# maiziezhoulab/FocalSV

Measured on AMD Instinct MI355X. Metric: target regions/sec (50 kb, 30x HiFi), higher is better.
Workload: dtype u32; 1 GPU; 256 synthetic 50 kb regions per GPU, 30x HiFi-like reads U(10k,20k), 0.2% error, seed 1000+i (BASELINE.json configs[1]); regions_per_gpu=256

## Files before the change

### focalsv_amd/csrc/aln.hip

```cpp
#include "k_sketch.h"
#include <algorithm>
#include <memory>
#include <cstdio>
#include <cstdlib>
#include <cstring>
#include <vector>

namespace {

#define ALN_AMAX 8192
#define ALN_CHAIN_STRIDE (ALN_AMAX + 8)
#define ALN_MAX_REC 5
#define ALN_MAJ_REC 3
#define ALN_SUP_MIN 200
#define ALN_SUB_OCC 2
#define ALN_SUB_PER 1500
#define ALN_EV_CAP 2048
#define ALN_CG_CAP 1024
#define NW_LDS_Q 3072
#define NW_NEG (-(1 << 29))

struct AlnHeader { int32_t qbeg, tbeg, qend, tend, n_events, n_chain, rev, status; uint32_t ev_off, pad; };
struct AlnEvent { int32_t qs, qe, ts, te; };
struct NwTask { uint32_t pair; int32_t qs, ql, ts, tl; uint32_t cg_off; uint64_t bt_off; uint64_t row_off; uint32_t out_idx, pad; };
// ... 675 lines not shown
__global__ __launch_bounds__(256) void k_nw_any(const uint32_t *__restrict__ store, const uint32_t *__restrict__ nm_all, const uint32_t *__restrict__ word_off,
                                                const int32_t *__restrict__ read_len, const uint32_t *__restrict__ pair_q,
                                                const uint32_t *__restrict__ pair_t, const AlnHeader *__restrict__ hdr,
                                                const NwTask *__restrict__ tasks, uint8_t *__restrict__ bt_all, int32_t *__restrict__ rows_all,
                                                uint32_t *__restrict__ cg_all, uint32_t *__restrict__ cg_n, int32_t *__restrict__ scores, fsv_aln_params P)
{
    const uint32_t *nm = nm_active(nm_all);
    __shared__ uint8_t s_bt[NW_TD][NW_TC];
    __shared__ int s_walk[8];
    const NwTask T = tasks[blockIdx.x];
    const uint32_t qw = word_off[pair_q[T.pair]], tw = word_off[pair_t[T.pair]];
    const int lenq = read_len[pair_q[T.pair]], rev = hdr[T.pair].rev;
    const int ql = T.ql, tl = T.tl;
    const bool two = P.q2 >= 0;
    const NwRows R{rows_all + T.row_off, ql};
    uint8_t *bt = bt_all + T.bt_off;
    for (int d = 0; d <= ql + tl - 2; d++) {
        const int jlo = max(0, d - (tl - 1)), jhi = min(ql - 1, d);
        for (int j = jlo + (int)threadIdx.x; j <= jhi; j += blockDim.x) {
            const int i = d - j;
            nw_cell(R, d, i, j, tbase(store, nm, tw, T.ts + i), qbase(store, qw, lenq, rev, T.qs + j), two, P, bt, ql);
        }
        __threadfence_block();
        __syncthreads();
    }
    if (threadIdx.x == 0) scores[T.out_idx] = R.H(ql + tl - 2)[ql - 1];
    nw_backtrack(bt, ql, tl, cg_all + T.cg_off, cg_n + T.out_idx, s_bt, s_walk);
}

struct NwLanes {
    hipStream_t side[3] = {nullptr, nullptr, nullptr};
    hipEvent_t fork = nullptr, join[3] = {nullptr, nullptr, nullptr};
    NwLanes() = default;
    NwLanes(const NwLanes &) = delete;
    NwLanes &operator=(const NwLanes &) = delete;
    ~NwLanes()
    {
        for (int i = 0; i < 3; i++) { if (side[i]) (void)hipStreamDestroy(side[i]); if (join[i]) (void)hipEventDestroy(join[i]); }
        if (fork) (void)hipEventDestroy(fork);
    }
    int ready(fsv_ctx *ctx)
    {
        if (fork) return FSV_OK;
        FSV_HIP(ctx, hipEventCreateWithFlags(&fork, hipEventDisableTiming));
        for (int i = 0; i < 3; i++) {
            FSV_HIP(ctx, hipStreamCreateWithFlags(&side[i], hipStreamNonBlocking));
            FSV_HIP(ctx, hipEventCreateWithFlags(&join[i], hipEventDisableTiming));
        }
        return FSV_OK;
    }
};

struct AlnWs {
    Dev<uint32_t> store, word_off, pair_q, pair_t, sk_ends, sk_low, sk_high, mz_off, mz_cnt, warn, ev_count, cg, cg_n;
    Dev<uint32_t> nmask;
    Dev<int32_t> len, rows, scores, gap_shift;
    Dev<char> ascii;
    Dev<uint64_t> asc_off, chain;
    Dev<uint8_t> wper, bt;
    Dev<uint16_t> thin;
    Dev<fsv_mz> mz;
    Dev<AlnHeader> hdr;
    Dev<AlnEvent> events, ev_packed;
    Dev<NwTask> tasks;
    Dev<GapQuery> gaps;
    Dev<BoxSrc> box_src;
    Dev<CornerTask> corner;
    Dev<int2> corner_out;
    fsv_aln_stats stats = {};
    NwLanes lanes;
    std::unique_ptr<AlnWs> sub;
    const uint32_t *nm() const { return nmask.p + FSV_NM_LEAD; }
};

void aln_ws_free(fsv_ctx *ctx)
{
    delete (AlnWs *)ctx->aln_ws;
    ctx->aln_ws = nullptr;
}

AlnWs *aln_ws_get(fsv_ctx *ctx)
{
    if (!ctx->aln_ws) { ctx->aln_ws = new AlnWs(); ctx->aln_ws_free = aln_ws_free; }
    return (AlnWs *)ctx->aln_ws;
}

#define PAIR_SEQS(W) (W).store.p, (W).nm(), (W).word_off.p, (W).len.p, (W).pair_q.p, (W).pair_t.p
template <class K, class... A> int launch_pair(fsv_ctx *ctx, const AlnWs &W, hipStream_t stream, K kern, size_t grid, uint32_t block, A... own)
{
    FSV_LAUNCH(ctx, stream, kern, dim3((uint32_t)grid), dim3(block), 0, PAIR_SEQS(W), W.hdr.p, own...);
    return FSV_OK;
}
template <bool SUB> int launch_chain_aln(fsv_ctx *ctx, const AlnWs &W, uint32_t np, uint32_t R, const fsv_aln_params &P)
{
    FSV_LAUNCH(ctx, ctx->stream, k_chain_aln<SUB>, dim3(np), dim3(64), 0, W.len.p, W.mz.p, W.mz_off.p, W.mz_cnt.p, W.pair_q.p, W.pair_t.p, W.chain.p, W.hdr.p, R, P);
    return FSV_OK;
}
template <bool SUB> int launch_events(fsv_ctx *ctx, const AlnWs &W, uint32_t ns, const fsv_aln_params &P)
{
    FSV_LAUNCH(ctx, ctx->stream, k_aln_events<SUB>, dim3(ns), dim3(256), 0, PAIR_SEQS(W), W.chain.p, W.hdr.p, W.events.p, W.ev_packed.p, W.ev_count.p, P);
    return FSV_OK;
}

template <class L, class F> int lay_out(fsv_ctx *ctx, const std::vector<L> &len, F unit, uint64_t slack, std::vector<uint32_t> &off)
{
    const size_t n = len.size();
    off.assign(n + 1, 0);
// ... 602 lines not shown
```

### focalsv_amd/csrc/asm.hip

```cpp
#include "asm_kernels.h"
#include "k_kmer.h"
#include "layout.h"
#include <algorithm>
#include <chrono>
#include <cstdio>
#include <cstdlib>
#include <cstring>
#include <vector>
#include <thread>
#include <atomic>

namespace {

enum { KN_SKETCH, KN_UNIQ, KN_CHAIN, KN_BPM, KN_RESCUE, KN_PATH_FAST, KN_PATH_DP, KN_CONSENSUS, KN_REPACK, KN_EXACT, KN_STITCH, KN_PARTITION, KN_BND, KN_BND_CONS, KN_COUNT,
       ST_SKETCH = KN_COUNT, ST_CHAIN, ST_VERIFY, ST_PATH, ST_CONSENSUS, ST_FINAL };
const char *const kn_names[KN_COUNT] = {"k_sketch", "k_uniq", "k_chain", "k5_bpm", "k_rescue_accept", "k_path_fast", "k_path_dp", "k_consensus",
                                        "k_repack", "k_exact", "k_stitch", "k_partition", "k_bnd_tasks", "k_bnd_consensus"};
enum { PASS_NONE = -1, PASS_WINDOWS, PASS_JUNCTIONS, PASS_BCIG, PASS_COUNT };

struct KTimes {
    struct Rec { int k; hipEvent_t a, b; uint64_t bytes; };
    std::vector<Rec> recs;
    std::vector<hipEvent_t> pool;
    size_t used = 0;
    std::vector<size_t> by[PASS_COUNT][KN_COUNT];
    hipEvent_t get() { if (used == pool.size()) { hipEvent_t e; (void)hipEventCreate(&e); pool.push_back(e); } return pool[used++]; }
    size_t begin(fsv_ctx *ctx, int k, uint64_t bytes) { Rec r{k, get(), get(), bytes}; (void)hipEventRecord(r.a, ctx->stream); recs.push_back(r); return recs.size() - 1; }
    void begin(fsv_ctx *ctx, int pass, int k, uint64_t bytes) { const size_t i = begin(ctx, k, bytes); if (pass != PASS_NONE) by[pass][k].push_back(i); }
    void end(fsv_ctx *ctx) { (void)hipEventRecord(recs.back().b, ctx->stream); }
    void end(fsv_ctx *ctx, size_t idx) { (void)hipEventRecord(recs[idx].b, ctx->stream); }
    uint64_t *bytes_of(int pass, int k, size_t round) { const auto &v = by[pass][k]; return round < v.size() ? &recs[v[round]].bytes : nullptr; }
    void reset() { recs.clear(); used = 0; for (auto &p : by) for (auto &v : p) v.clear(); }
    ~KTimes() { for (auto e : pool) (void)hipEventDestroy(e); }
};

struct Span {
    fsv_ctx *ctx; KTimes &kt; size_t idx;
    Span(fsv_ctx *c, KTimes &k, int stage) : ctx(c), kt(k), idx(k.begin(c, stage, 0)) {}
    void stop() { kt.end(ctx, idx); }
};

enum { CT_TASKS = 0, CT_OVERFLOW = 1, CT_DP = 2, CT_INEXACT = 3, CT_COLS_LO = 4, CT_COLS_HI = 5, CT_DP_WIDE = 6, CT_DP_SB = 7, CT_DP_GEN = 8, CT_DP_XW = 9,
       CT_MZ_LO = 10, CT_MZ_HI = 11, CT_B_RETRY = 12, CT_B_LIST = 13, CT_DP_SB16 = 14, CT_WIDE = 15,
       CT_MZRAW_LO = 16, CT_MZRAW_HI = 17, CT_BASES_LO = 18, CT_BASES_HI = 19,
       CT_DP_FR3 = 20,
       CT_LEFT = 21,
       CT_FIX = 22, CT_FIXED = 23,
       CT_SLOT = 24 };

template <class... Ts> size_t cap_sum(const Ts &...b) { return (b.cap + ... + 0); }

struct AsmWs {
    Dev<uint32_t> store[2], word_off, set_start, read_set, pair_base, upair_base, pair_read, mz_off, mz_cnt, counters, warn, set_cols, changed, read_dirty,
        dp_list, dp_list2, dp_list3, dp_list16, dp_list_e3, dp_wide, dp_xwide, left_list, fix_list, wide_list, inexact_list, cols_wide,
        gwin_off, gwin_read, lb, unpack_off, brel_off, src3, bnd_flag, bnd_list, site_cnt, site_off, redo, sk_ends, sk_low, sk_high;
    Dev<uint32_t> sr_store;
    Dev<uint32_t> site_cursor;
    Dev<uint32_t> site_lists;
    Dev<uint32_t> set_hits;
    Dev<int32_t> len, new_len, idx2, bc_idx;
    Dev<int32_t> bc_win;
    Dev<fsv_mz> mz; Dev<fsv_ovl> ovl, ovl_prev; Dev<fsv_hit> hits, hits_packed; Dev<fsv_piece> pieces; Dev<BndPatch> bnd_patch;
    Dev<fsv_wtask> tasks, tasks2, tasks3; Dev<fsv_wres> res, res2, res3; Dev<fsv_wpath> paths, paths2;
    Dev<uint4> cols_sb, ovl_c, upair_tab, upair_tab_sw, gwin_tab, bc_rec; Dev<uint2> site_rec; Dev<int8_t> site_vec;
    Dev<uint64_t> cols;
    Dev<unsigned long long> tmp;
    Dev<uint8_t> cov3, bnd_bytes, exact_flag, cwin, thr_tab; Dev<uint16_t> cwin_len; Dev<char> contig_out, contig_all;
    Dev<unsigned long long> km_keys, km_flt, km_flt_all; Dev<uint32_t> km_cnt, km_hist, km_cursor, km_err; Dev<uint64_t> km_tab_off, km_flt_off;
    Dev<int32_t> km_cutoff; Dev<KmerTile> km_tiles;
    Dev<unsigned long long> fs_keys, fs_list; Dev<uint64_t> fs_off, fs_list_off; Dev<uint32_t> fs_read_set;
    SketchFilter flt;
    std::vector<fsv_kmer_index_set> ki_last; double ki_ms = 0; bool ki_valid = false;
    Dev<fsv_wtask> ext_tasks; Dev<fsv_wext> ext_res; Dev<uint32_t> ext_list, charge_list, charge_n; Dev<unsigned long long> charge_ct;
    std::vector<hipEvent_t> charge_ev;
    fsv_charge_stats charge_last{};
    bool charge_valid = false;
    std::vector<fsv_kmer_set> km_last; std::vector<uint64_t> km_last_flt_off; const unsigned long long *km_last_flt = nullptr; double km_ms = 0; bool km_valid = false;
    std::vector<uint32_t> h_store;
    int occ_sb = 0, occ_fr[3] = {0, 0, 0}, occ_wide = 0;
    ChainArgs last_chain;
    std::vector<uint32_t> h_word_off;
    std::vector<int32_t> h_len;
    const uint32_t *cur_store = nullptr;
    uint32_t n_reads = 0;
    fsv_asm_stats stats;
    KTimes kt;
    void *h_pin = nullptr; size_t h_pin_cap = 0;
    uint32_t *ct_of(int row) { return counters.p + (size_t)row * CT_SLOT; }
    size_t held() const
    {
        return cap_sum(store[0], store[1], cols_sb, contig_all, word_off, len, set_start, read_set, pair_base, mz, mz_off, mz_cnt, ovl, tasks, res, paths,
                       counters, dp_list, dp_list2, dp_list3, dp_list16, dp_list_e3, dp_wide, dp_xwide, cols_wide, set_cols, site_cnt, site_rec, site_off, site_vec,
                       site_cursor, redo, site_lists, read_dirty, cov3, lb, sr_store, brel_off, tasks2, res2, paths2, idx2, bc_idx, bc_rec, bc_win, left_list, fix_list,
                       tasks3, res3, src3, bnd_flag, bnd_list, bnd_patch, bnd_bytes, changed, pair_read, wide_list, cols, tmp, gwin_off, gwin_read, sk_ends, sk_low, sk_high,
                       hits, hits_packed, set_hits, ovl_prev, exact_flag, inexact_list, upair_base, upair_tab, upair_tab_sw, ovl_c, gwin_tab, cwin, cwin_len, warn, thr_tab,
                       pieces, contig_out, new_len, unpack_off, km_keys, km_flt, km_flt_all, km_cnt, km_hist, km_cursor, km_err, km_tab_off, km_flt_off, km_cutoff, km_tiles,
                       fs_keys, fs_list, fs_off, fs_list_off, fs_read_set, ext_tasks, ext_res, ext_list, charge_list, charge_n, charge_ct);
    }
};

void ws_free(fsv_ctx *ctx)
{
    AsmWs *w = (AsmWs *)ctx->asm_ws;
    if (!w) return;
    if (w->h_pin) (void)hipHostFree(w->h_pin);
    for (auto e : w->charge_ev) (void)hipEventDestroy(e);
    delete w;
    ctx->asm_ws = nullptr;
}

AsmWs *ws_get(fsv_ctx *ctx)
{
    if (!ctx->asm_ws) { ctx->asm_ws = new AsmWs(); ctx->asm_ws_free = ws_free; memset(&((AsmWs *)ctx->asm_ws)->stats, 0, sizeof(fsv_asm_stats)); }
    return (AsmWs *)ctx->asm_ws;
}

uint8_t thr_for_len_host(int x_len, int rate_pm)
{
    const double rate = rate_pm / 1000.0;
    if (x_len == FSV_WINDOW) return rate_pm == 40 ? FSV_K_FULL : (uint8_t)(int)(FSV_WINDOW * rate);
    int t = (int)(x_len * rate);
    if (t == 0 && x_len >= 4) t = 1;
    return (uint8_t)t;
}

struct Batch {
    uint32_t n_reads = 0, n_sets = 0, n_pairs = 0, n_upairs = 0;
    std::vector<uint32_t> set_start, read_set, pair_base, upair_base;
};

struct Geometry {
    std::vector<uint32_t> word_off, mz_off, gwin_off, gwin_read;
    uint64_t task_bound = 0;
    uint32_t max_words = 1;
};

static inline uint64_t mz_slots(int64_t len, int) { return (uint64_t)len + 64; }

int make_geometry(fsv_ctx *ctx, const Batch &B, const std::vector<int32_t> &len, Geometry &G, int mz_w = 51, const std::vector<uint32_t> *fixed_mz_off = nullptr)
{
    G.word_off.assign(B.n_reads + 1, 0); G.mz_off.assign(B.n_reads + 1, 0); G.gwin_off.assign(B.n_reads + 1, 0);
    G.max_words = 1;
    uint64_t w = 0, m = 0, g = 0;
    for (uint32_t r = 0; r < B.n_reads; r++) {
        G.word_off[r] = (uint32_t)w; G.mz_off[r] = (uint32_t)m; G.gwin_off[r] = (uint32_t)g;
        w += (uint64_t)(len[r] + 15) / 16;
        G.max_words = std::max<uint32_t>(G.max_words, (uint32_t)((len[r] + 15) / 16));
// ... 1394 lines not shown
}

static int check_asm_params(fsv_ctx *ctx, const fsv_asm_params &P)
{
    if (P.k < 1 || P.k > 63 || P.w < 1 || P.w > 64 || P.lookback != 64 || P.n_rounds < 0 || P.n_rounds > 16 || P.min_anchors < 1)
        return fsv_fail(ctx, FSV_EINVAL, "fsv_asm_params out of range (k<=63, w<=64, lookback==64)");
    if (P.k_cap < 1 || P.k_cap > FSV_K_WIDE || P.win_rate_pm < 1 || (int)(FSV_WINDOW * (P.win_rate_pm / 1000.0)) > P.k_cap || P.accept_err_pm < 0 || P.accept_err_pm > 1000 ||
        P.w_later < 0 || P.w_later > 64)
        return fsv_fail(ctx, FSV_EINVAL, "fsv_asm_params error model out of range (k_cap <= 95, 375 x win_rate_pm / 1000 <= k_cap)");
    if (P.kmer_filter && !P.kmer_table)
        return fsv_fail(ctx, FSV_EINVAL, "kmer_filter = 1 needs kmer_table = 1: the filter is the list the k-mer count table stage leaves");
    if (P.partial_charge && P.k_cap > FSV_K_MAX)
        return fsv_fail(ctx, FSV_EINVAL, "partial_charge needs k_cap <= 31 (FSV_K_MAX): the charge is not restated for the wide-band profiles");
    return FSV_OK;
}

static int fsv_assemble_batch_impl(fsv_ctx *ctx, const fsv_readsets *sets, const fsv_asm_params *params, fsv_contigs *out)
{
    if (!ctx || !sets || !out || !sets->store_dev || !sets->word_off || !sets->read_len || !sets->set_start) return FSV_EINVAL;
    if (!out->seq || !out->off || !out->set || !out->n_reads || !out->set_status) return FSV_EINVAL;
    fsv_asm_params P;
    if (params) P = *params; else fsv_asm_default_params(&P);
    TRY(check_asm_params(ctx, P));
    FSV_HIP(ctx, hipSetDevice(ctx->device));
    AsmWs &W = *ws_get(ctx);
    out->n_contigs = 0; out->off[0] = 0;
    W.km_last.clear(); W.km_last_flt_off.assign(1, 0); W.km_last_flt = nullptr; W.km_ms = 0; W.km_valid = false;
    W.flt = SketchFilter{}; W.ki_last.clear(); W.ki_ms = 0; W.ki_valid = false;
    W.charge_last = fsv_charge_stats{}; W.charge_valid = false;
    for (auto e : W.charge_ev) (void)hipEventDestroy(e);
    W.charge_ev.clear();
    if (sets->n_sets == 0 || (sets->n_reads == 0 && !P.kmer_table)) { for (uint32_t s = 0; s < sets->n_sets; s++) out->set_status[s] = 0; memset(&W.stats, 0, sizeof(W.stats)); W.charge_valid = P.partial_charge != 0; return FSV_OK; }
    if (sets->set_start[0] != 0 || sets->set_start[sets->n_sets] != sets->n_reads) return fsv_fail(ctx, FSV_EINVAL, "set_start must span [0, n_reads]");
    for (uint32_t s = 0; s < sets->n_sets; s++) if (sets->set_start[s + 1] < sets->set_start[s]) return fsv_fail(ctx, FSV_EINVAL, "set_start not monotone");
    const char *env = getenv("FSV_ASM_BUDGET_GB");
    double budget = 0.4 * (double)ctx->hbm_bytes;
    {
        size_t free_b = 0, total_b = 0;
        const size_t own = W.held();
        if (hipMemGetInfo(&free_b, &total_b) == hipSuccess)
            budget = std::min(budget, 0.9 * ((double)free_b / (double)std::max(1, fsv_live_contexts(ctx->device)) + (double)own));
    }
    if (env && atof(env) > 0) budget = atof(env) * 1e9;
    std::vector<uint32_t> cut{0};
    {
        uint64_t tk = 0, pr = 0, bs = 0, km = 0;
        for (uint32_t s = 0; s < sets->n_sets; s++) {
            uint64_t t1, p1, b1, k1, f1;
            set_cost(sets, s, t1, p1, b1, k1, f1);
            if (!P.kmer_table) k1 = 0;
            if (P.kmer_filter) k1 += f1;
            if (t1 >= (1ull << 31) || p1 >= (1ull << 31) || b1 + b1 / 4 >= (1ull << 32)) return fsv_fail(ctx, FSV_EUNSUP, "a single read set exceeds the 2^31 window-task / pair bound");
            const bool over = tk + t1 >= (1ull << 31) || pr + p1 >= (1ull << 31) || (bs + b1) + (bs + b1) / 4 >= (1ull << 32) ||
                              (double)(tk + t1) * (P.second_round ? 400.0 : 200.0) + (double)(pr + p1) * 200.0 + (double)(bs + b1) * (P.second_round ? 52.0 : 48.0) +
                              (double)(km + k1) + (P.partial_charge ? (double)(tk + t1) * 104.0 : 0.0) > budget;
            if (over && s > cut.back()) { cut.push_back(s); tk = pr = bs = km = 0; }
            tk += t1; pr += p1; bs += b1; km += k1;
        }
        cut.push_back(sets->n_sets);
    }
    if (cut.size() == 2) { TRY(assemble_chunk(ctx, sets, P, out)); W.km_valid = P.kmer_table != 0; W.ki_valid = P.kmer_filter != 0; W.charge_valid = P.partial_charge != 0; return FSV_OK; }
    fsv_asm_stats total; memset(&total, 0, sizeof(total));
    uint64_t used = 0; uint32_t nc = 0;
    std::vector<uint64_t> all_off{0};
    for (size_t c = 0; c + 1 < cut.size(); c++) {
        const uint32_t s0 = cut[c], s1 = cut[c + 1], r0 = sets->set_start[s0], r1 = sets->set_start[s1];
        std::vector<uint32_t> sub_start(s1 - s0 + 1);
        for (uint32_t s = s0; s <= s1; s++) sub_start[s - s0] = sets->set_start[s] - r0;
        fsv_readsets sub = *sets;
        std::vector<uint64_t> sub_woff((size_t)(r1 - r0) + 1);
        for (uint32_t r = r0; r <= r1; r++) sub_woff[r - r0] = sets->word_off[r] - sets->word_off[r0];
        sub.store_dev = sets->store_dev + sets->word_off[r0];
        sub.word_off = sub_woff.data(); sub.read_len = sets->read_len + r0; sub.set_start = sub_start.data();
        sub.n_reads = r1 - r0; sub.n_sets = s1 - s0; sub.set_flags = sets->set_flags ? sets->set_flags + s0 : nullptr;
        fsv_contigs part = *out;
        part.seq = out->seq + used; part.seq_cap = out->seq_cap - used; part.off = out->off + nc; part.set = out->set + nc; part.n_reads = out->n_reads + nc;
        part.contig_cap = out->contig_cap - nc; part.set_status = out->set_status + s0; part.n_contigs = 0;
        const uint64_t keep = out->off[nc];
        TRY(assemble_chunk(ctx, &sub, P, &part));
        out->off[nc] = keep;
        for (uint32_t i = 0; i < part.n_contigs; i++) { out->set[nc + i] += s0; out->off[nc + i + 1] += used; }
        const uint64_t bytes = part.n_contigs ? out->off[nc + part.n_contigs] - used : 0;
        if (bytes) {
            if (W.contig_all.cap < used + bytes + 16) {
                Dev<char> bigger;
                TRY(ensure(ctx, bigger, std::max<uint64_t>((used + bytes) * 2, 1u << 20)));
                if (used) FSV_HIP(ctx, hipMemcpyAsync(bigger.p, W.contig_all.p, used, hipMemcpyDeviceToDevice, ctx->stream));
                FSV_HIP(ctx, hipStreamSynchronize(ctx->stream));
                W.contig_all.swap(bigger);
            }
            FSV_HIP(ctx, hipMemcpyAsync(W.contig_all.p + used, W.contig_out.p, bytes, hipMemcpyDeviceToDevice, ctx->stream));
        }
        used += bytes; nc += part.n_contigs;
        const fsv_asm_stats &st = W.stats;
        total.n_pairs += st.n_pairs; total.n_overlaps += st.n_overlaps; total.n_windows += st.n_windows; total.n_windows_matched += st.n_windows_matched;
        total.n_paths += st.n_paths; total.n_path_dp += st.n_path_dp; total.dp_columns += st.dp_columns; total.algo_bytes += st.algo_bytes;
        total.n_exact_overlaps += st.n_exact_overlaps; total.n_inexact_candidates += st.n_inexact_candidates; total.n_path_fr += st.n_path_fr;
        total.ms_sketch += st.ms_sketch; total.ms_chain += st.ms_chain; total.ms_verify += st.ms_verify; total.ms_path += st.ms_path;
        total.ms_consensus += st.ms_consensus; total.ms_final += st.ms_final; total.ms_total += st.ms_total;
        total.n_kernels = st.n_kernels;
        for (uint32_t k = 0; k < st.n_kernels; k++) {
            memcpy(total.kernels[k].name, st.kernels[k].name, sizeof(st.kernels[k].name));
            total.kernels[k].ms += st.kernels[k].ms; total.kernels[k].launches += st.kernels[k].launches; total.kernels[k].algo_bytes += st.kernels[k].algo_bytes;
        }
    }
    FSV_HIP(ctx, hipStreamSynchronize(ctx->stream));
    out->n_contigs = nc;
// ... 218 lines not shown
```

### focalsv_amd/csrc/k_sketch.h

```cpp
#pragma once
#include "fsv_internal.h"

#define FSV_UQ_MAX     4096

namespace {

__device__ __forceinline__ uint64_t mix64(uint64_t key)
{
    key = ~key + (key << 21);
    key = key ^ key >> 24;
    key = (key + (key << 3)) + (key << 8);
    key = key ^ key >> 14;
    key = (key + (key << 2)) + (key << 4);
    key = key ^ key >> 28;
    key = key + (key << 31);
    return key;
}

#ifndef FSV_KMER_EMPTY
#define FSV_KMER_EMPTY (~0ull)
#endif
template <bool FLT> struct FltView {};
template <> struct FltView<true> { const unsigned long long *keys; const uint64_t *off; const uint32_t *read_set; };
struct SketchFilter { const unsigned long long *keys = nullptr; const uint64_t *off = nullptr; const uint32_t *read_set = nullptr; };
// ... 220 lines not shown
    __syncthreads();
    const uint32_t m = mz_cnt[r];
    const uint32_t o0 = s_scan[tid];
    const uint32_t slot_cap = mz_off[r + 1] - mz_off[r];
    __syncthreads();
#pragma unroll
    for (uint32_t j = 0; j < UQ_MAX / 256; j++)
        if (j < cnt) { s_hash[o0 + j] = kh[j]; s_pay[o0 + j] = kp[j]; }
    __syncthreads();
    for (uint32_t i = tid; i < m; i += 256) { fsv_mz x; x.hash = s_hash[i]; const uint64_t p = s_pay[i]; x.pos = (uint32_t)p; x.rev = (uint8_t)(p >> 32); x.span = (uint8_t)(p >> 40); x.pad = 0; a[i] = x; }
    if (2 * m <= slot_cap) {
        uint32_t mp = 1;
        while (mp < m) mp <<= 1;
        for (uint32_t i = m + tid; i < mp; i += 256) { s_hash[i] = ~0ull; s_pay[i] = ~0ull; }
        __syncthreads();
        for (uint32_t sz = 2; sz <= mp; sz <<= 1)
            for (uint32_t st = sz >> 1; st > 0; st >>= 1) {
                for (uint32_t t = tid; t < mp / 2; t += 256) {
                    const uint32_t i = ((t & ~(st - 1)) << 1) | (t & (st - 1)), j = i | st;
                    const bool up = (i & sz) == 0;
                    const uint64_t pi = s_pay[i], pj = s_pay[j];
                    bool gt = (uint32_t)pi > (uint32_t)pj || ((uint32_t)pi == (uint32_t)pj && pi > pj);
                    if (pi == ~0ull && pj != ~0ull) gt = true; else if (pj == ~0ull) gt = false;
                    if (gt == up) { const uint64_t hi2 = s_hash[i], hj = s_hash[j]; s_hash[i] = hj; s_hash[j] = hi2; s_pay[i] = pj; s_pay[j] = pi; }
                }
                __syncthreads();
            }
        for (uint32_t i = tid; i < m; i += 256) { fsv_mz x; x.hash = s_hash[i]; const uint64_t p = s_pay[i]; x.pos = (uint32_t)p; x.rev = (uint8_t)(p >> 32); x.span = (uint8_t)(p >> 40); x.pad = 0; a[m + i] = x; }
    } else if (tid == 0) atomicOr(&warn[r], (uint32_t)FSV_W_INTERNAL);
}

template <int UQ_MAX>
__global__ __launch_bounds__(256) void k_uniq(fsv_mz *__restrict__ mz, const uint32_t *__restrict__ mz_off, uint32_t *__restrict__ mz_cnt,
                                              uint32_t *__restrict__ warn, const uint32_t *__restrict__ only_changed = nullptr,
                                              uint32_t lo_cnt = 0u, uint32_t hi_cnt = 0xffffffffu, unsigned long long *__restrict__ total = nullptr,
                                              uint32_t max_occ = 1u)
{
    uniq_read<UQ_MAX>(blockIdx.x, mz, mz_off, mz_cnt, warn, only_changed, lo_cnt, hi_cnt, total, max_occ);
}

template <int UQ_MAX>
__global__ __launch_bounds__(256) void k_uniq_walk(fsv_mz *__restrict__ mz, const uint32_t *__restrict__ mz_off, uint32_t *__restrict__ mz_cnt,
                                                   uint32_t *__restrict__ warn, const uint32_t *__restrict__ only_changed, uint32_t lo_cnt, uint32_t hi_cnt,
                                                   unsigned long long *__restrict__ total, uint32_t n_reads)
{
    for (uint32_t r = blockIdx.x; r < n_reads; r += gridDim.x) {
        uniq_read<UQ_MAX>(r, mz, mz_off, mz_cnt, warn, only_changed, lo_cnt, hi_cnt, total);
        __syncthreads();
    }
}

#define SKF_T 1024
#define SKF_V ((SKF_T + 2 * 256 + 255) / 256)
template <bool FLT>
__global__ __launch_bounds__(256) void k_sketch_fast(const uint32_t *__restrict__ store, const uint32_t *__restrict__ word_off,
                                                     const int32_t *__restrict__ read_len, const uint32_t *__restrict__ mz_off,
                                                     fsv_mz *__restrict__ mz, uint32_t *__restrict__ mz_cnt, uint32_t n_reads, int w, int k,
                                                     int hpc, uint32_t *__restrict__ warn, const uint8_t *__restrict__ w_per_read,
                                                     uint32_t *__restrict__ sc_ends, uint32_t *__restrict__ sc_low, uint32_t *__restrict__ sc_high,
                                                     const uint32_t *__restrict__ only_changed, const FltView<FLT> F)
{
    __shared__ uint64_t s_h[SKF_T + 2 * 256];
    __shared__ uint64_t s_wmin[SKF_T + 2 * 256];
    __shared__ uint32_t s_scan[4];
    __shared__ uint32_t s_carry;
    __shared__ uint64_t s_am, s_ah;
    __shared__ int s_abest, s_short;
    const int tid = threadIdx.x;
    const uint32_t r = blockIdx.x;
    if (r >= n_reads) return;
    if (only_changed && !only_changed[r]) return;
    const uint32_t woff = word_off[r];
    const int len = read_len[r];
    const uint32_t cap = mz_off[r + 1] - mz_off[r];
    fsv_mz *out = mz + mz_off[r];
    if (w_per_read) w = w_per_read[r];
    [[maybe_unused]] uint64_t fbase = 0, fsize = 0;
    if constexpr (FLT) { const uint32_t fs = F.read_set[r]; fbase = F.off[fs]; fsize = F.off[fs + 1] - fbase; }
    if (tid == 0) mz_cnt[r] = 0;
    uint32_t *ends = sc_ends + (size_t)woff * 16;
    uint32_t *low = sc_low + woff + r, *high = sc_high + woff + r;
    const uint64_t NONE = ~0ull;
    const uint64_t kmask = (1ull << k) - 1;
    const int nwords = (len + 15) >> 4;
    if (tid == 0) s_carry = 0;
    __syncthreads();
    for (int wbase = 0; wbase < nwords; wbase += 256) {
        const int wi = wbase + tid;
        uint32_t flags = 0, word = 0;
        int nb = 0;
        if (wi < nwords) {
            word = store[woff + wi];
            nb = min(16, len - wi * 16);
            if (hpc) {
                const uint32_t nextb = (wi + 1 < nwords) ? (store[woff + wi + 1] & 3u) : 4u;
                const uint32_t shifted = (word >> 2) | (nextb << 30);
                uint32_t d = word ^ shifted;
                d = (d | (d >> 1)) & 0x55555555u;
                d = (d | (d >> 1)) & 0x33333333u; d = (d | (d >> 2)) & 0x0f0f0f0fu; d = (d | (d >> 4)) & 0x00ff00ffu; d = (d | (d >> 8)) & 0xffffu;
                flags = nb >= 16 ? d : (d & ((1u << nb) - 1u));
                if (len - 1 - wi * 16 < 16) flags |= 1u << (len - 1 - wi * 16);
            } else flags = nb >= 16 ? 0xffffu : ((1u << nb) - 1u);
        }
        const uint32_t cnt = __popc(flags);
        uint32_t incl = cnt;
        for (int off = 1; off < 64; off <<= 1) { const uint32_t o2 = __shfl_up(incl, off, 64); if ((tid & 63) >= off) incl += o2; }
        if ((tid & 63) == 63) s_scan[tid >> 6] = incl;
        __syncthreads();
        uint32_t wave_before = 0, tile_total = 0;
#pragma unroll
        for (int wv = 0; wv < 4; wv++) { const uint32_t v = s_scan[wv]; if (wv < (tid >> 6)) wave_before += v; tile_total += v; }
        const uint32_t base = s_carry + wave_before + incl - cnt;
        if (cnt) {
            uint32_t lo = 0, hi = 0, rank = 0;
            for (int j = 0; j < nb; j++)
                if ((flags >> j) & 1u) {
                    const uint32_t b = (word >> (2 * j)) & 3u;
                    lo |= (b & 1u) << rank; hi |= (b >> 1) << rank;
                    ends[base + rank] = (uint32_t)(wi * 16 + j);
                    rank++;
                }
            const uint32_t wd = base >> 5, sh = base & 31u;
            atomicOr(&low[wd], lo << sh); atomicOr(&high[wd], hi << sh);
            if (sh + cnt > 32) { atomicOr(&low[wd + 1], lo >> (32 - sh)); atomicOr(&high[wd + 1], hi >> (32 - sh)); }
        }
        __syncthreads();
        if (tid == 0) s_carry += tile_total;
        __syncthreads();
    }
    const int M = (int)s_carry;
    const int T0 = w + k - 2;
    __threadfence_block();
    __syncthreads();
    auto cut = [&](const uint32_t *pl, int a) -> uint64_t {
        const int wd = a >> 5, sh = a & 31;
        const uint64_t lo64 = (uint64_t)pl[wd] | (uint64_t)pl[wd + 1] << 32;
        uint64_t v = lo64 >> sh;
        if (sh) v |= (uint64_t)pl[wd + 2] << (64 - sh);
        return v & kmask;
    };
    auto entry_hash = [&](int e, int *z_out) -> uint64_t {
        if (e < k - 1 || e >= M) return NONE;
        const int span = (int)ends[e] - (e - k >= 0 ? (int)ends[e - k] : -1);
        if (hpc && span >= 256) return NONE;
        const uint64_t lo = cut(low, e - k + 1), hi = cut(high, e - k + 1);
        const uint64_t f0 = __brevll(lo) >> (64 - k), f1 = __brevll(hi) >> (64 - k);
        const uint64_t r0 = ~lo & kmask, r1 = ~hi & kmask;
        const int z = f1 < r1 ? 0 : 1;
        if (z_out) *z_out = z;
        const uint64_t h = mix64(z ? r0 : f0) + mix64(z ? r1 : f1);
        if constexpr (FLT) if (fsize && flt_has(F.keys, fbase, fsize, h)) return NONE;
        return h;
    };
    auto emit = [&](int p) {
        int z = 0;
        const uint64_t h = entry_hash(p, &z);
        const int span = hpc ? (int)ends[p] - (p - k >= 0 ? (int)ends[p - k] : -1) : k;
        const uint32_t at = atomicAdd(&mz_cnt[r], 1u);
        if (at < cap) { fsv_mz m; m.hash = h; m.pos = ends[p]; m.rev = (uint8_t)z; m.span = (uint8_t)span; m.pad = 0; out[at] = m; }
        else atomicOr(&warn[r], (uint32_t)FSV_W_MZ_TRUNC);
    };
    for (int t0 = 0; t0 < M; t0 += SKF_T) {
        const int e0 = t0 - (w - 1);
        for (int idx = tid; idx < SKF_T + 2 * (w - 1); idx += 256) s_h[idx] = entry_hash(e0 + idx, nullptr);
        __syncthreads();
        const int NW = SKF_T + 2 * (w - 1);
        int p2 = 1;
        while (p2 * 2 <= w) p2 <<= 1;
        uint64_t v[SKF_V];
#pragma unroll
        for (int c = 0; c < SKF_V; c++) { const int i = tid + 256 * c; v[c] = i < NW ? s_h[i] : NONE; }
        auto pass = [&](const uint64_t *src, int d, bool is_max) {
#pragma unroll
            for (int c = 0; c < SKF_V; c++) {
                const int i = tid + 256 * c;
                if (i < NW) {
                    const uint64_t b = i + d < NW ? src[i + d] : (is_max ? 0ull : NONE);
                    v[c] = is_max ? max(v[c], b) : min(v[c], b);
                }
            }
            __syncthreads();
#pragma unroll
            for (int c = 0; c < SKF_V; c++) { const int i = tid + 256 * c; if (i < NW) s_wmin[i] = v[c]; }
            __syncthreads();
        };
        if (w == 1) pass(s_h, 0, false);
        else {
            pass(s_h, 1, false);
            for (int d = 2; d < p2; d <<= 1) pass(s_wmin, d, false);
            if (w > p2) pass(s_wmin, w - p2, false);
        }
        if (t0 == 0 && tid == 0) {
            s_short = -1; s_abest = -1; s_am = NONE; s_ah = NONE;
            if (M <= T0) {
                uint64_t m = NONE; int bp = -1;
                for (int p = max(0, M - w); p < M; p++) { const uint64_t h = s_h[p - e0]; if (h != NONE && h <= m) { m = h; bp = p; } }
                s_short = bp;
            } else {
                uint64_t m = NONE; int bp = -1;
                for (int p = T0 - w + 1; p <= T0 - 1; p++) { const uint64_t h = s_h[p - e0]; if (h != NONE && h <= m) { m = h; bp = p; } }
                s_am = m; s_abest = bp; s_ah = s_h[T0 - e0];
            }
        }
        __syncthreads();
        if (M > T0) {
            {
#pragma unroll
                for (int c = 0; c < SKF_V; c++) {
                    const int i = tid + 256 * c, t = t0 + i;
                    if (i < NW && !(t >= T0 && t <= M - 1 && i < SKF_T + w - 1)) { s_wmin[i] = 0ull; v[c] = 0ull; }
                }
                __syncthreads();
            }
            if (w > 1) {
                for (int d = 1; d < p2; d <<= 1) pass(s_wmin, d, true);
                if (w > p2) pass(s_wmin, w - p2, true);
            }
        }
        for (int pi = tid; pi < SKF_T; pi += 256) {
            const int p = t0 + pi;
            if (p >= M) break;
            const uint64_t hp = s_h[pi + (w - 1)];
            if (hp == NONE) continue;
            bool e;
            if (M <= T0) e = (p == s_short);
            else {
                e = (p + w - 1 >= T0) && s_wmin[pi] == hp;
                if (p >= T0 - w + 1 && p <= T0 - 1 && s_am != NONE && hp == s_am) e = (p != s_abest) ? true : (s_ah > s_am);
            }
            if (e) emit(p);
        }
        __syncthreads();
    }
}

struct SketchJob {
    const uint32_t *store; uint32_t n_reads; size_t total_words; uint32_t max_words;
    int w, k, hpc; const uint8_t *wper; int w_max;
    bool replay;
    const uint32_t *only_changed;
    SketchFilter flt = {};
};
template <class Ws> int launch_sketch(fsv_ctx *ctx, Ws &W, const SketchJob &J)
{
    const bool fast = (J.k & 1) && !J.replay;
    if (!(fast && J.only_changed)) TRY(zero(ctx, W.mz_cnt, J.n_reads));
    if (fast) {
        const size_t plane = J.total_words + J.n_reads + 8;
        TRY(ensure(ctx, W.sk_ends, J.total_words * 16 + 64));
        TRY(ensure_each(ctx, plane, W.sk_low, W.sk_high));
        TRY(zero(ctx, W.sk_low, plane));
        TRY(zero(ctx, W.sk_high, plane));
        if (J.flt.keys)
            FSV_LAUNCH(ctx, ctx->stream, k_sketch_fast<true>, dim3(J.n_reads), dim3(256), 0, J.store, W.word_off.p, W.len.p, W.mz_off.p, W.mz.p, W.mz_cnt.p,
                       J.n_reads, J.w, J.k, J.hpc, W.warn.p, J.wper, W.sk_ends.p, W.sk_low.p, W.sk_high.p, J.only_changed, FltView<true>{J.flt.keys, J.flt.off, J.flt.read_set});
        else
            FSV_LAUNCH(ctx, ctx->stream, k_sketch_fast<false>, dim3(J.n_reads), dim3(256), 0, J.store, W.word_off.p, W.len.p, W.mz_off.p, W.mz.p, W.mz_cnt.p,
                       J.n_reads, J.w, J.k, J.hpc, W.warn.p, J.wper, W.sk_ends.p, W.sk_low.p, W.sk_high.p, J.only_changed, FltView<false>{});
    } else {
        const uint32_t lds_words = J.max_words < 8192u ? J.max_words : 8192u;
        const size_t lds = sketch_lds_bytes(J.w_max, lds_words);
        if (J.flt.keys) {
            FSV_HIP(ctx, hipFuncSetAttribute((const void *)k_sketch<true>, hipFuncAttributeMaxDynamicSharedMemorySize, (int)lds));
            FSV_LAUNCH(ctx, ctx->stream, k_sketch<true>, dim3(J.n_reads), dim3(64), lds, J.store, W.word_off.p, W.len.p, W.mz_off.p, W.mz.p, W.mz_cnt.p,
                       J.n_reads, J.w, J.k, J.hpc, W.warn.p, J.wper, J.w_max, lds_words, FltView<true>{J.flt.keys, J.flt.off, J.flt.read_set});
        } else {
            FSV_HIP(ctx, hipFuncSetAttribute((const void *)k_sketch<false>, hipFuncAttributeMaxDynamicSharedMemorySize, (int)lds));
            FSV_LAUNCH(ctx, ctx->stream, k_sketch<false>, dim3(J.n_reads), dim3(64), lds, J.store, W.word_off.p, W.len.p, W.mz_off.p, W.mz.p, W.mz_cnt.p,
                       J.n_reads, J.w, J.k, J.hpc, W.warn.p, J.wper, J.w_max, lds_words, FltView<false>{});
        }
    }
    return FSV_OK;
}

}
```

Measured before the change: 2515 regions/s.

## Rebuild sketch base planes per tile in LDS instead of global scratch

The fast minimizer sketch kernel no longer writes per-base end positions and 2-bit low/high planes to global scratch. It stores only a per-word prefix count, then rebuilds the ends and bit planes for each tile in shared memory before hashing. This removes the large global scratch buffers, their zeroing memsets and the global atomics. It also merges the hash and window-min buffers into one LDS array, keeps hashes in registers, and pins occupancy at 8 waves per EU. The cost is recomputing word flags per tile, more LDS atomics, and a slightly smaller per-base budget estimate in the batch-splitting heuristic.

```diff
diff --git a/focalsv_amd/csrc/aln.hip b/focalsv_amd/csrc/aln.hip
--- a/focalsv_amd/csrc/aln.hip
+++ b/focalsv_amd/csrc/aln.hip
@@ -751,7 +751,7 @@
 };
 
 struct AlnWs {
-    Dev<uint32_t> store, word_off, pair_q, pair_t, sk_ends, sk_low, sk_high, mz_off, mz_cnt, warn, ev_count, cg, cg_n;
+    Dev<uint32_t> store, word_off, pair_q, pair_t, sk_pre, mz_off, mz_cnt, warn, ev_count, cg, cg_n;
     Dev<uint32_t> nmask;
     Dev<int32_t> len, rows, scores, gap_shift;
     Dev<char> ascii;
diff --git a/focalsv_amd/csrc/asm.hip b/focalsv_amd/csrc/asm.hip
--- a/focalsv_amd/csrc/asm.hip
+++ b/focalsv_amd/csrc/asm.hip
@@ -53,7 +53,7 @@
 struct AsmWs {
     Dev<uint32_t> store[2], word_off, set_start, read_set, pair_base, upair_base, pair_read, mz_off, mz_cnt, counters, warn, set_cols, changed, read_dirty,
         dp_list, dp_list2, dp_list3, dp_list16, dp_list_e3, dp_wide, dp_xwide, left_list, fix_list, wide_list, inexact_list, cols_wide,
-        gwin_off, gwin_read, lb, unpack_off, brel_off, src3, bnd_flag, bnd_list, site_cnt, site_off, redo, sk_ends, sk_low, sk_high;
+        gwin_off, gwin_read, lb, unpack_off, brel_off, src3, bnd_flag, bnd_list, site_cnt, site_off, redo, sk_pre;
     Dev<uint32_t> sr_store;
     Dev<uint32_t> site_cursor;
     Dev<uint32_t> site_lists;
@@ -92,7 +92,7 @@
         return cap_sum(store[0], store[1], cols_sb, contig_all, word_off, len, set_start, read_set, pair_base, mz, mz_off, mz_cnt, ovl, tasks, res, paths,
                        counters, dp_list, dp_list2, dp_list3, dp_list16, dp_list_e3, dp_wide, dp_xwide, cols_wide, set_cols, site_cnt, site_rec, site_off, site_vec,
                        site_cursor, redo, site_lists, read_dirty, cov3, lb, sr_store, brel_off, tasks2, res2, paths2, idx2, bc_idx, bc_rec, bc_win, left_list, fix_list,
-                       tasks3, res3, src3, bnd_flag, bnd_list, bnd_patch, bnd_bytes, changed, pair_read, wide_list, cols, tmp, gwin_off, gwin_read, sk_ends, sk_low, sk_high,
+                       tasks3, res3, src3, bnd_flag, bnd_list, bnd_patch, bnd_bytes, changed, pair_read, wide_list, cols, tmp, gwin_off, gwin_read, sk_pre,
                        hits, hits_packed, set_hits, ovl_prev, exact_flag, inexact_list, upair_base, upair_tab, upair_tab_sw, ovl_c, gwin_tab, cwin, cwin_len, warn, thr_tab,
                        pieces, contig_out, new_len, unpack_off, km_keys, km_flt, km_flt_all, km_cnt, km_hist, km_cursor, km_err, km_tab_off, km_flt_off, km_cutoff, km_tiles,
                        fs_keys, fs_list, fs_off, fs_list_off, fs_read_set, ext_tasks, ext_res, ext_list, charge_list, charge_n, charge_ct);
@@ -1593,7 +1593,7 @@
             if (P.kmer_filter) k1 += f1;
             if (t1 >= (1ull << 31) || p1 >= (1ull << 31) || b1 + b1 / 4 >= (1ull << 32)) return fsv_fail(ctx, FSV_EUNSUP, "a single read set exceeds the 2^31 window-task / pair bound");
             const bool over = tk + t1 >= (1ull << 31) || pr + p1 >= (1ull << 31) || (bs + b1) + (bs + b1) / 4 >= (1ull << 32) ||
-                              (double)(tk + t1) * (P.second_round ? 400.0 : 200.0) + (double)(pr + p1) * 200.0 + (double)(bs + b1) * (P.second_round ? 52.0 : 48.0) +
+                              (double)(tk + t1) * (P.second_round ? 400.0 : 200.0) + (double)(pr + p1) * 200.0 + (double)(bs + b1) * (P.second_round ? 48.0 : 44.0) +
                               (double)(km + k1) + (P.partial_charge ? (double)(tk + t1) * 104.0 : 0.0) > budget;
             if (over && s > cut.back()) { cut.push_back(s); tk = pr = bs = km = 0; }
             tk += t1; pr += p1; bs += b1; km += k1;
diff --git a/focalsv_amd/csrc/k_sketch.h b/focalsv_amd/csrc/k_sketch.h
--- a/focalsv_amd/csrc/k_sketch.h
+++ b/focalsv_amd/csrc/k_sketch.h
@@ -296,16 +296,19 @@
 
 #define SKF_T 1024
 #define SKF_V ((SKF_T + 2 * 256 + 255) / 256)
+#define SKF_E (SKF_T + 2 * 254 + 63 + 1)
+#define SKF_P ((SKF_E + 31) / 32 + 3)
 template <bool FLT>
-__global__ __launch_bounds__(256) void k_sketch_fast(const uint32_t *__restrict__ store, const uint32_t *__restrict__ word_off,
-                                                     const int32_t *__restrict__ read_len, const uint32_t *__restrict__ mz_off,
-                                                     fsv_mz *__restrict__ mz, uint32_t *__restrict__ mz_cnt, uint32_t n_reads, int w, int k,
-                                                     int hpc, uint32_t *__restrict__ warn, const uint8_t *__restrict__ w_per_read,
-                                                     uint32_t *__restrict__ sc_ends, uint32_t *__restrict__ sc_low, uint32_t *__restrict__ sc_high,
-                                                     const uint32_t *__restrict__ only_changed, const FltView<FLT> F)
-{
-    __shared__ uint64_t s_h[SKF_T + 2 * 256];
-    __shared__ uint64_t s_wmin[SKF_T + 2 * 256];
+__global__ __launch_bounds__(256) __attribute__((amdgpu_waves_per_eu(8, 8)))
+void k_sketch_fast(const uint32_t *__restrict__ store, const uint32_t *__restrict__ word_off,
+                   const int32_t *__restrict__ read_len, const uint32_t *__restrict__ mz_off,
+                   fsv_mz *__restrict__ mz, uint32_t *__restrict__ mz_cnt, uint32_t n_reads, int w, int k,
+                   int hpc, uint32_t *__restrict__ warn, const uint8_t *__restrict__ w_per_read, uint32_t *__restrict__ sc_pre,
+                   const uint32_t *__restrict__ only_changed, const FltView<FLT> F)
+{
+    __shared__ uint64_t s_t[SKF_T + 2 * 256];
+    __shared__ uint32_t s_ends[SKF_E];
+    __shared__ uint32_t s_low[SKF_P], s_high[SKF_P];
     __shared__ uint32_t s_scan[4];
     __shared__ uint32_t s_carry;
     __shared__ uint64_t s_am, s_ah;
@@ -322,31 +325,29 @@
     [[maybe_unused]] uint64_t fbase = 0, fsize = 0;
     if constexpr (FLT) { const uint32_t fs = F.read_set[r]; fbase = F.off[fs]; fsize = F.off[fs + 1] - fbase; }
     if (tid == 0) mz_cnt[r] = 0;
-    uint32_t *ends = sc_ends + (size_t)woff * 16;
-    uint32_t *low = sc_low + woff + r, *high = sc_high + woff + r;
+    uint32_t *pre = sc_pre + woff + r;
     const uint64_t NONE = ~0ull;
     const uint64_t kmask = (1ull << k) - 1;
     const int nwords = (len + 15) >> 4;
+    auto word_flags = [&](int wi, uint32_t &word) -> uint32_t {
+        word = store[woff + wi];
+        const int nb = min(16, len - wi * 16);
+        if (!hpc) return nb >= 16 ? 0xffffu : ((1u << nb) - 1u);
+        const uint32_t nextb = (wi + 1 < nwords) ? (store[woff + wi + 1] & 3u) : 4u;
+        const uint32_t shifted = (word >> 2) | (nextb << 30);
+        uint32_t d = word ^ shifted;
+        d = (d | (d >> 1)) & 0x55555555u;
+        d = (d | (d >> 1)) & 0x33333333u; d = (d | (d >> 2)) & 0x0f0f0f0fu; d = (d | (d >> 4)) & 0x00ff00ffu; d = (d | (d >> 8)) & 0xffffu;
+        uint32_t flags = nb >= 16 ? d : (d & ((1u << nb) - 1u));
+        if (len - 1 - wi * 16 < 16) flags |= 1u << (len - 1 - wi * 16);
+        return flags;
+    };
     if (tid == 0) s_carry = 0;
     __syncthreads();
     for (int wbase = 0; wbase < nwords; wbase += 256) {
         const int wi = wbase + tid;
-        uint32_t flags = 0, word = 0;
-        int nb = 0;
-        if (wi < nwords) {
-            word = store[woff + wi];
-            nb = min(16, len - wi * 16);
-            if (hpc) {
-                const uint32_t nextb = (wi + 1 < nwords) ? (store[woff + wi + 1] & 3u) : 4u;
-                const uint32_t shifted = (word >> 2) | (nextb << 30);
-                uint32_t d = word ^ shifted;
-                d = (d | (d >> 1)) & 0x55555555u;
-                d = (d | (d >> 1)) & 0x33333333u; d = (d | (d >> 2)) & 0x0f0f0f0fu; d = (d | (d >> 4)) & 0x00ff00ffu; d = (d | (d >> 8)) & 0xffffu;
-                flags = nb >= 16 ? d : (d & ((1u << nb) - 1u));
-                if (len - 1 - wi * 16 < 16) flags |= 1u << (len - 1 - wi * 16);
-            } else flags = nb >= 16 ? 0xffffu : ((1u << nb) - 1u);
-        }
-        const uint32_t cnt = __popc(flags);
+        uint32_t word = 0;
+        const uint32_t cnt = wi < nwords ? __popc(word_flags(wi, word)) : 0u;
         uint32_t incl = cnt;
         for (int off = 1; off < 64; off <<= 1) { const uint32_t o2 = __shfl_up(incl, off, 64); if ((tid & 63) >= off) incl += o2; }
         if ((tid & 63) == 63) s_scan[tid >> 6] = incl;
@@ -354,20 +355,7 @@
         uint32_t wave_before = 0, tile_total = 0;
 #pragma unroll
         for (int wv = 0; wv < 4; wv++) { const uint32_t v = s_scan[wv]; if (wv < (tid >> 6)) wave_before += v; tile_total += v; }
-        const uint32_t base = s_carry + wave_before + incl - cnt;
-        if (cnt) {
-            uint32_t lo = 0, hi = 0, rank = 0;
-            for (int j = 0; j < nb; j++)
-                if ((flags >> j) & 1u) {
-                    const uint32_t b = (word >> (2 * j)) & 3u;
-                    lo |= (b & 1u) << rank; hi |= (b >> 1) << rank;
-                    ends[base + rank] = (uint32_t)(wi * 16 + j);
-                    rank++;
-                }
-            const uint32_t wd = base >> 5, sh = base & 31u;
-            atomicOr(&low[wd], lo << sh); atomicOr(&high[wd], hi << sh);
-            if (sh + cnt > 32) { atomicOr(&low[wd + 1], lo >> (32 - sh)); atomicOr(&high[wd + 1], hi >> (32 - sh)); }
-        }
+        if (wi < nwords) pre[wi] = s_carry + wave_before + incl - cnt;
         __syncthreads();
         if (tid == 0) s_carry += tile_total;
         __syncthreads();
@@ -376,8 +364,9 @@
     const int T0 = w + k - 2;
     __threadfence_block();
     __syncthreads();
+    int lo = 0;
     auto cut = [&](const uint32_t *pl, int a) -> uint64_t {
-        const int wd = a >> 5, sh = a & 31;
+        const int wd = (a - lo) >> 5, sh = (a - lo) & 31;
         const uint64_t lo64 = (uint64_t)pl[wd] | (uint64_t)pl[wd + 1] << 32;
         uint64_t v = lo64 >> sh;
         if (sh) v |= (uint64_t)pl[wd + 2] << (64 - sh);
@@ -385,11 +374,11 @@
     };
     auto entry_hash = [&](int e, int *z_out) -> uint64_t {
         if (e < k - 1 || e >= M) return NONE;
-        const int span = (int)ends[e] - (e - k >= 0 ? (int)ends[e - k] : -1);
+        const int span = (int)s_ends[e - lo] - (e - k >= 0 ? (int)s_ends[e - k - lo] : -1);
         if (hpc && span >= 256) return NONE;
-        const uint64_t lo = cut(low, e - k + 1), hi = cut(high, e - k + 1);
-        const uint64_t f0 = __brevll(lo) >> (64 - k), f1 = __brevll(hi) >> (64 - k);
-        const uint64_t r0 = ~lo & kmask, r1 = ~hi & kmask;
+        const uint64_t b0 = cut(s_low, e - k + 1), b1 = cut(s_high, e - k + 1);
+        const uint64_t f0 = __brevll(b0) >> (64 - k), f1 = __brevll(b1) >> (64 - k);
+        const uint64_t r0 = ~b0 & kmask, r1 = ~b1 & kmask;
         const int z = f1 < r1 ? 0 : 1;
         if (z_out) *z_out = z;
         const uint64_t h = mix64(z ? r0 : f0) + mix64(z ? r1 : f1);
@@ -399,81 +388,121 @@
     auto emit = [&](int p) {
         int z = 0;
         const uint64_t h = entry_hash(p, &z);
-        const int span = hpc ? (int)ends[p] - (p - k >= 0 ? (int)ends[p - k] : -1) : k;
+        const uint32_t end = s_ends[p - lo];
+        const int span = hpc ? (int)end - (p - k >= 0 ? (int)s_ends[p - k - lo] : -1) : k;
         const uint32_t at = atomicAdd(&mz_cnt[r], 1u);
-        if (at < cap) { fsv_mz m; m.hash = h; m.pos = ends[p]; m.rev = (uint8_t)z; m.span = (uint8_t)span; m.pad = 0; out[at] = m; }
+        if (at < cap) { fsv_mz m; m.hash = h; m.pos = end; m.rev = (uint8_t)z; m.span = (uint8_t)span; m.pad = 0; out[at] = m; }
         else atomicOr(&warn[r], (uint32_t)FSV_W_MZ_TRUNC);
     };
+    int cur = 0;
     for (int t0 = 0; t0 < M; t0 += SKF_T) {
         const int e0 = t0 - (w - 1);
-        for (int idx = tid; idx < SKF_T + 2 * (w - 1); idx += 256) s_h[idx] = entry_hash(e0 + idx, nullptr);
-        __syncthreads();
         const int NW = SKF_T + 2 * (w - 1);
-        int p2 = 1;
-        while (p2 * 2 <= w) p2 <<= 1;
-        uint64_t v[SKF_V];
-#pragma unroll
-        for (int c = 0; c < SKF_V; c++) { const int i = tid + 256 * c; v[c] = i < NW ? s_h[i] : NONE; }
-        auto pass = [&](const uint64_t *src, int d, bool is_max) {
-#pragma unroll
-            for (int c = 0; c < SKF_V; c++) {
-                const int i = tid + 256 * c;
-                if (i < NW) {
-                    const uint64_t b = i + d < NW ? src[i + d] : (is_max ? 0ull : NONE);
-                    v[c] = is_max ? max(v[c], b) : min(v[c], b);
+        lo = max(0, e0 - k);
+        const int hi = min(M, e0 + NW);
+        for (int i = tid; i < SKF_P; i += 256) { s_low[i] = 0u; s_high[i] = 0u; }
+        __syncthreads();
+        for (int wc = cur, found = 0;; wc += 256) {
+            const int wi = wc + tid;
+            int base = M, cnt = 0;
+            if (wi < nwords) {
+                uint32_t word;
+                uint32_t flags = word_flags(wi, word);
+                base = (int)pre[wi]; cnt = __popc(flags);
+                if (base < hi && base + cnt > lo) {
+                    uint32_t bl = 0, bh = 0;
+                    for (int rank = 0; flags; flags &= flags - 1, rank++) {
+                        const int j = __ffs(flags) - 1, e = base + rank;
+                        const uint32_t b = (word >> (2 * j)) & 3u;
+                        bl |= (b & 1u) << rank; bh |= (b >> 1) << rank;
+                        if (e >= lo && e < hi) s_ends[e - lo] = (uint32_t)(wi * 16 + j);
+                    }
+                    int off = base - lo;
+                    if (off < 0) { bl >>= -off; bh >>= -off; off = 0; }
+                    const int wd = off >> 5, sh = off & 31;
+                    if (bl << sh) atomicOr(&s_low[wd], bl << sh);
+                    if (bh << sh) atomicOr(&s_high[wd], bh << sh);
+                    if (sh > 16) { if (bl >> (32 - sh)) atomicOr(&s_low[wd + 1], bl >> (32 - sh)); if (bh >> (32 - sh)) atomicOr(&s_high[wd + 1], bh >> (32 - sh)); }
                 }
             }
-            __syncthreads();
-#pragma unroll
-            for (int c = 0; c < SKF_V; c++) { const int i = tid + 256 * c; if (i < NW) s_wmin[i] = v[c]; }
-            __syncthreads();
-        };
-        if (w == 1) pass(s_h, 0, false);
-        else {
-            pass(s_h, 1, false);
-            for (int d = 2; d < p2; d <<= 1) pass(s_wmin, d, false);
-            if (w > p2) pass(s_wmin, w - p2, false);
-        }
+            if (!found) { const int skip = __syncthreads_count(wi < nwords && base + cnt <= lo); cur = wc + skip; found = skip < 256; }
+            if (wc + 256 >= nwords || (int)pre[wc + 256] >= hi) break;
+        }
+        __syncthreads();
+        uint64_t hreg[SKF_V];
+#pragma unroll
+        for (int c = 0; c < SKF_V; c++) {
+            const int i = tid + 256 * c;
+            hreg[c] = NONE;
+            if (i < NW) { hreg[c] = entry_hash(e0 + i, nullptr); s_t[i] = hreg[c]; }
+        }
+        __syncthreads();
         if (t0 == 0 && tid == 0) {
             s_short = -1; s_abest = -1; s_am = NONE; s_ah = NONE;
             if (M <= T0) {
                 uint64_t m = NONE; int bp = -1;
-                for (int p = max(0, M - w); p < M; p++) { const uint64_t h = s_h[p - e0]; if (h != NONE && h <= m) { m = h; bp = p; } }
+                for (int p = max(0, M - w); p < M; p++) { const uint64_t h = s_t[p - e0]; if (h != NONE && h <= m) { m = h; bp = p; } }
                 s_short = bp;
             } else {
                 uint64_t m = NONE; int bp = -1;
-                for (int p = T0 - w + 1; p <= T0 - 1; p++) { const uint64_t h = s_h[p - e0]; if (h != NONE && h <= m) { m = h; bp = p; } }
-                s_am = m; s_abest = bp; s_ah = s_h[T0 - e0];
-            }
-        }
-        __syncthreads();
+                for (int p = T0 - w + 1; p <= T0 - 1; p++) { const uint64_t h = s_t[p - e0]; if (h != NONE && h <= m) { m = h; bp = p; } }
+                s_am = m; s_abest = bp; s_ah = s_t[T0 - e0];
+            }
+        }
+        int p2 = 1;
+        while (p2 * 2 <= w) p2 <<= 1;
+        uint64_t v[SKF_V];
+#pragma unroll
+        for (int c = 0; c < SKF_V; c++) v[c] = hreg[c];
+        auto pass = [&](int d, bool is_max) {
+#pragma unroll
+            for (int c = 0; c < SKF_V; c++) {
+                const int i = tid + 256 * c;
+                if (i < NW) {
+                    const uint64_t b = i + d < NW ? s_t[i + d] : (is_max ? 0ull : NONE);
+                    v[c] = is_max ? max(v[c], b) : min(v[c], b);
+                }
+            }
+            __syncthreads();
+#pragma unroll
+            for (int c = 0; c < SKF_V; c++) { const int i = tid + 256 * c; if (i < NW) s_t[i] = v[c]; }
+            __syncthreads();
+        };
+        if (w == 1) pass(0, false);
+        else {
+            for (int d = 1; d < p2; d <<= 1) pass(d, false);
+            if (w > p2) pass(w - p2, false);
+        }
         if (M > T0) {
             {
 #pragma unroll
                 for (int c = 0; c < SKF_V; c++) {
                     const int i = tid + 256 * c, t = t0 + i;
-                    if (i < NW && !(t >= T0 && t <= M - 1 && i < SKF_T + w - 1)) { s_wmin[i] = 0ull; v[c] = 0ull; }
+                    if (i < NW && !(t >= T0 && t <= M - 1 && i < SKF_T + w - 1)) { s_t[i] = 0ull; v[c] = 0ull; }
                 }
                 __syncthreads();
             }
             if (w > 1) {
-                for (int d = 1; d < p2; d <<= 1) pass(s_wmin, d, true);
-                if (w > p2) pass(s_wmin, w - p2, true);
-            }
-        }
-        for (int pi = tid; pi < SKF_T; pi += 256) {
-            const int p = t0 + pi;
-            if (p >= M) break;
-            const uint64_t hp = s_h[pi + (w - 1)];
+                for (int d = 1; d < p2; d <<= 1) pass(d, true);
+                if (w > p2) pass(w - p2, true);
+            }
+        }
+        uint32_t hits = 0;
+#pragma unroll
+        for (int c = 0; c < SKF_V; c++) {
+            const int i = tid + 256 * c, pi = i - (w - 1), p = t0 + pi;
+            if (pi < 0 || pi >= SKF_T || p >= M) continue;
+            const uint64_t hp = hreg[c];
             if (hp == NONE) continue;
             bool e;
             if (M <= T0) e = (p == s_short);
             else {
-                e = (p + w - 1 >= T0) && s_wmin[pi] == hp;
+                e = (p + w - 1 >= T0) && s_t[pi] == hp;
                 if (p >= T0 - w + 1 && p <= T0 - 1 && s_am != NONE && hp == s_am) e = (p != s_abest) ? true : (s_ah > s_am);
             }
-            if (e) emit(p);
-        }
+            if (e) hits |= 1u << c;
+        }
+        for (; hits; hits &= hits - 1) emit(e0 + tid + 256 * (__ffs(hits) - 1));
         __syncthreads();
     }
 }
@@ -490,17 +519,13 @@
     const bool fast = (J.k & 1) && !J.replay;
     if (!(fast && J.only_changed)) TRY(zero(ctx, W.mz_cnt, J.n_reads));
     if (fast) {
-        const size_t plane = J.total_words + J.n_reads + 8;
-        TRY(ensure(ctx, W.sk_ends, J.total_words * 16 + 64));
-        TRY(ensure_each(ctx, plane, W.sk_low, W.sk_high));
-        TRY(zero(ctx, W.sk_low, plane));
-        TRY(zero(ctx, W.sk_high, plane));
+        TRY(ensure(ctx, W.sk_pre, J.total_words + J.n_reads + 8));
         if (J.flt.keys)
             FSV_LAUNCH(ctx, ctx->stream, k_sketch_fast<true>, dim3(J.n_reads), dim3(256), 0, J.store, W.word_off.p, W.len.p, W.mz_off.p, W.mz.p, W.mz_cnt.p,
-                       J.n_reads, J.w, J.k, J.hpc, W.warn.p, J.wper, W.sk_ends.p, W.sk_low.p, W.sk_high.p, J.only_changed, FltView<true>{J.flt.keys, J.flt.off, J.flt.read_set});
+                       J.n_reads, J.w, J.k, J.hpc, W.warn.p, J.wper, W.sk_pre.p, J.only_changed, FltView<true>{J.flt.keys, J.flt.off, J.flt.read_set});
         else
             FSV_LAUNCH(ctx, ctx->stream, k_sketch_fast<false>, dim3(J.n_reads), dim3(256), 0, J.store, W.word_off.p, W.len.p, W.mz_off.p, W.mz.p, W.mz_cnt.p,
-                       J.n_reads, J.w, J.k, J.hpc, W.warn.p, J.wper, W.sk_ends.p, W.sk_low.p, W.sk_high.p, J.only_changed, FltView<false>{});
+                       J.n_reads, J.w, J.k, J.hpc, W.warn.p, J.wper, W.sk_pre.p, J.only_changed, FltView<false>{});
     } else {
         const uint32_t lds_words = J.max_words < 8192u ? J.max_words : 8192u;
         const size_t lds = sketch_lds_bytes(J.w_max, lds_words);
```

Result: no change. 2506 regions/s (-0.4%).
